# LSDOlab/femo_alpha

Measured on AMD Instinct MI355X. Metric: DOF/s (assembly+solve), forward solve of the RM shell; adjoint-gradient wallclock in adjoint_ms, higher is better.
Workload: dtype f64

## Files before the change

### femo_alpha_amd/backend.py

```python
from __future__ import annotations

import ctypes as C

import numpy as np

from . import _lib
from ._lib import FemoHipError, dptr, iptr
from .mesh import ShellMesh

PENALTY_BETA = 1.0e15


class FemoConvergenceError(FemoHipError):
    """A Krylov solve stopped at maxit short of rtol (status 4; option 'strict')."""


class FemoNotPositiveDefiniteError(FemoHipError):
    """The multifrontal Cholesky met a non-positive pivot (status 5; option 'allow_pivot_repair')."""


class ShellContext:
    VEC_IDS = {"state": 0, "adjoint": 1, "r": 2, "z": 3, "p": 4, "Ap": 5, "b": 6}

    def __init__(self, mesh: ShellMesh, element_wise_material=False, elementwise_pressure=False,
# ... 8 lines not shown
        h = C.c_void_p()
        xyz = np.ascontiguousarray(mesh.nodes, dtype=np.float64)
        cells = np.ascontiguousarray(mesh.cells, dtype=np.int32)
        cp2 = np.ascontiguousarray(mesh.cell_p2, dtype=np.int32)
        if getattr(mesh, "element", "CG2CG1") == "CG2CR1":
            rc = self.lib.femo_create_element(C.byref(h), int(device), mesh.nn, mesh.nel, mesh.nvc, mesh.nP2,
                                              dptr(xyz), iptr(cells), iptr(cp2),
                                              int(self.element_wise_material), int(self.elementwise_pressure), int(nquad),
                                              int(nghost), 1)
        else:
            rc = self.lib.femo_create_ghost(C.byref(h), int(device), mesh.nn, mesh.nel, mesh.nvc, mesh.nP2,
                                            dptr(xyz), iptr(cells), iptr(cp2),
                                            int(self.element_wise_material), int(self.elementwise_pressure), int(nquad),
                                            int(nghost))
        if rc:
            raise FemoHipError(f"femo_create failed ({rc}): {self.lib.femo_last_error(None).decode()}")
        self._h = h
        self.device = int(device)
        self.nghost = int(nghost)
        self.ndof = int(self.lib.femo_ndof(h))
        assert self.ndof == mesh.ndof + self.nghost
        import os
        self.env_options = {}
        for kv in filter(None, (t.strip() for t in os.environ.get("FEMO_OPTIONS", "").split(","))):
            k, sep, v = kv.partition("=")
            try:
                if not sep:
                    raise ValueError
                self.env_options[k.strip()] = float(v)
            except ValueError:
                raise FemoHipError(f"FEMO_OPTIONS: '{kv}' is not of the form option=number (e.g. FEMO_OPTIONS=\"sweep_graph=1,super_tiles=1\")") from None
            self.set_option(k.strip(), self.env_options[k.strip()])
        if self.env_options:
            import sys
            print(f"femo_alpha_amd: FEMO_OPTIONS sets {self.env_options} on this context", file=sys.stderr)

    def _chk(self, rc):
        if rc:
            msg = self.lib.femo_last_error(self._h).decode()
            if rc == 4:
                raise FemoConvergenceError(msg)
            if rc == 5:
                raise FemoNotPositiveDefiniteError(msg)
            raise FemoHipError(msg)

    def set_option(self, key, value):
        self._chk(self.lib.femo_set_option(self._h, key.encode(), float(value)))

    def close(self):
        if getattr(self, "_h", None):
            self.lib.femo_destroy(self._h)
            self._h = None

    def __del__(self):
        try:
            self.close()
        except Exception:
            pass

    @staticmethod
    def _vec(a):
        return np.ascontiguousarray(np.asarray(a, dtype=np.float64).ravel())

    def field_size(self, name):
        n = int(self.lib.femo_field_size(self._h, name.encode()))
        if n < 0:
            raise FemoHipError(f"unknown field '{name}'")
        return n

# ... 156 lines not shown
        wp = None if w is None else dptr(self._vec(w))
        self._chk(self.lib.femo_residual(self._h, wp, dptr(r)))
        return r

    def load_vector(self):
        F = np.empty(self.ndof)
        self._chk(self.lib.femo_load_vector(self._h, dptr(F)))
        return F

    def diagonal(self):
        d = np.empty(self.ndof)
        self._chk(self.lib.femo_diagonal(self._h, dptr(d)))
        return d

    def element_matrices(self, first=0, count=None):
        count = self.mesh.nel - first if count is None else count
        ld = self.mesh.ldof
        Ke = np.empty((count, ld, ld))
        self._chk(self.lib.femo_element_matrices(self._h, first, count, dptr(Ke)))
        return Ke

    def enable_frontal(self, leaf_size=None, plan=None, **options):
        import time
        from .solver.symbolic import build_plan
        leaf_size = self.mesh.recommended_leaf_size() if leaf_size is None else int(leaf_size)
        for k, v in options.items():
            self.set_option(k, v)
        t0 = time.perf_counter()
        plan = self.plan = build_plan(self.mesh, leaf_size) if plan is None else plan
        self.symbolic_s = time.perf_counter() - t0
        i32 = lambda a: np.ascontiguousarray(a, dtype=np.int32)
        i64 = lambda a: np.ascontiguousarray(a, dtype=np.int64)
        level_off = i32(np.concatenate([[0], np.cumsum([len(l) for l in plan.level_nodes])]))
        level_nodes = i32(np.concatenate(plan.level_nodes))
        arrs = dict(nf=i32(plan.nf), npiv=i32(plan.npiv), front_off=i64(plan.front_off), dof_off=i64(plan.dof_off),
                    front_dofs=i32(plan.front_dofs), up_map=i32(plan.up_map), parent=i32(plan.parent), left=i32(plan.left),
                    right=i32(plan.right), level_off=level_off, level_nodes=level_nodes,
                    elem_front=i32(plan.elem_front), elem_map=i32(plan.elem_map))
        p64 = lambda a: a.ctypes.data_as(C.POINTER(C.c_int64))
        self._chk(self.lib.femo_set_frontal_plan(
            self._h, plan.ntree, plan.nlevels, iptr(arrs["nf"]), iptr(arrs["npiv"]), p64(arrs["front_off"]),
            p64(arrs["dof_off"]), iptr(arrs["front_dofs"]), iptr(arrs["up_map"]), iptr(arrs["parent"]), iptr(arrs["left"]),
            iptr(arrs["right"]), iptr(arrs["level_off"]), iptr(arrs["level_nodes"]), iptr(arrs["elem_front"]),
            iptr(arrs["elem_map"])))
        return plan

    def factorize(self):
        self._chk(self.lib.femo_factorize(self._h))
        return self.frontal_info()

    def factorize_profile(self, run=True):
        t = np.zeros(32)
# ... 502 lines not shown
```

### femo_alpha_amd/csrc/symbolic.cpp

```cpp
#include <omp.h>

#include <algorithm>
#include <cmath>
#include <cstdint>
#include <cstdlib>
#include <cstring>
#include <map>
#include <numeric>
#include <string>
#include <vector>

#include "../../include/femo_symbolic.h"

namespace {

struct Plan {
    std::map<std::string, std::vector<int32_t>> i32;
    std::map<std::string, std::vector<int64_t>> i64;
    std::string error;
};

thread_local std::string g_error;

template <class T>
std::vector<T>& put(std::map<std::string, std::vector<T>>& m, const char* name) { return m[name]; }

}

struct femo_plan : Plan {};

extern "C" {

const char* femo_plan_last_error(void) { return g_error.c_str(); }

void femo_plan_free(femo_plan* p) { delete p; }

int femo_plan_build_ex(femo_plan** out, int32_t nel, int32_t nP2, int32_t nV, int32_t npc, int32_t ndpc, const int32_t* cell_p2,
                       const double* cent, const double* cext, const int32_t* cell_dofs, int32_t leaf_size, int32_t min_depth,
                       int32_t axis_rule, double gap_coeff) {
    return femo_plan_build_ex2(out, nel, nP2, nV, npc, ndpc, cell_p2, cent, cext, cell_dofs, leaf_size, min_depth, axis_rule, gap_coeff, 0);
}

int femo_plan_build_ex2(femo_plan** out, int32_t nel, int32_t nP2, int32_t nV, int32_t npc, int32_t ndpc, const int32_t* cell_p2,
                        const double* cent, const double* cext, const int32_t* cell_dofs, int32_t leaf_size, int32_t min_depth,
                        int32_t axis_rule, double gap_coeff, int32_t node_order) {
    if (!out || node_order < 0 || node_order > 1 || nel < 1 || nP2 < 1 || nV < 1 || npc < 1 || ndpc < 1 || !cell_p2 || !cent || !cell_dofs || leaf_size < 1 || min_depth < 0 ||
        axis_rule < 0 || axis_rule > 2 || (axis_rule >= 1 && !cext) || !(gap_coeff >= 0.0)) {
        g_error = "femo_plan_build: bad arguments";
        return 1;
    }
    const int nthreads = std::max(1, std::min(omp_get_max_threads(), 16));
    const int64_t ndof_u = 3 * (int64_t)nP2;
    int32_t fixed_depth = 0;
    while (((int64_t)leaf_size << fixed_depth) < (int64_t)nel) ++fixed_depth;
    fixed_depth = std::max(fixed_depth, min_depth);
    const bool gap_mode = gap_coeff > 0.0;
    constexpr int32_t GAP_NMIN = 128;
    constexpr int32_t AXIS_NMIN = 16;
    std::vector<int32_t> lo{0}, hi{nel}, left{-1}, right{-1}, parent{-1}, depth{0};
    std::vector<int32_t> eorder(nel);
    std::iota(eorder.begin(), eorder.end(), 0);
    struct Scratch { std::vector<int32_t> stamp, first, last, touched; std::vector<long long> diff; };
    std::vector<Scratch> scratch(nthreads);
    {
        std::vector<int32_t> frontier{0};
        while (!frontier.empty()) {
            std::vector<int32_t> split(frontier.size(), -1);
            int bad = 0;
#pragma omp parallel for num_threads(nthreads) schedule(dynamic, 1) reduction(| : bad)
// ... 173 lines not shown
        for (int32_t d = maxdepth; d >= 0; --d) {
            const auto& nodes = by_depth[d];
#pragma omp parallel for num_threads(nthreads) schedule(dynamic, 16)
            for (int64_t k = 0; k < (int64_t)nodes.size(); ++k) {
                const int32_t t = nodes[k];
                std::vector<int32_t> u;
                if (left[t] < 0) {
                    for (int32_t i = lo[t]; i < hi[t]; ++i)
                        for (int a = 0; a < npc; ++a) u.push_back(cell_p2[(int64_t)eorder[i] * npc + a]);
                    std::sort(u.begin(), u.end());
                    u.erase(std::unique(u.begin(), u.end()), u.end());
                } else {
                    const auto &x = bnd[left[t]], &y = bnd[right[t]];
                    u.resize(x.size() + y.size());
                    u.erase(std::set_union(x.begin(), x.end(), y.begin(), y.end(), u.begin()), u.end());
                }
                auto& b = bnd[t];
                b.reserve(u.size());
                for (int32_t n : u)
                    if (owner[n] != t) b.push_back(n);
            }
        }
    }
    if (node_order == 1) {
#pragma omp parallel for num_threads(nthreads) schedule(dynamic, 64)
        for (int32_t t = 0; t < ntree; ++t)
            std::sort(bnd[t].begin(), bnd[t].end(), [&](int32_t x, int32_t y) {
                const int32_t dx = depth[owner[x]], dy = depth[owner[y]];
                return dx != dy ? dx > dy : rank[x] < rank[y];
            });
    }
    std::vector<int64_t> bnd_off(ntree + 1, 0);
    for (int32_t t = 0; t < ntree; ++t) bnd_off[t + 1] = bnd_off[t] + (int64_t)bnd[t].size();
    std::vector<int32_t> bnd_nodes(bnd_off[ntree]);
    for (int32_t t = 0; t < ntree; ++t) std::copy(bnd[t].begin(), bnd[t].end(), bnd_nodes.begin() + bnd_off[t]);
    auto ndofs_of = [&](int32_t n) { return n < nV ? 6 : 3; };
    std::vector<int32_t> npiv(ntree), nf(ntree);
    std::vector<int64_t> dof_off(ntree + 1, 0);
    for (int32_t t = 0; t < ntree; ++t) {
        int64_t a = 0, b = 0;
        for (int64_t i = piv_off[t]; i < piv_off[t + 1]; ++i) a += ndofs_of(piv_nodes[i]);
        for (int32_t n : bnd[t]) b += ndofs_of(n);
        if (a + b > INT32_MAX) { g_error = "front too large"; return 4; }
        npiv[t] = (int32_t)a; nf[t] = (int32_t)(a + b);
        dof_off[t + 1] = dof_off[t] + a + b;
    }
    if (ndof_u + 3 * (int64_t)nV > INT32_MAX) { g_error = "more than 2^31 DOFs"; return 4; }
    std::vector<int32_t> front_dofs(dof_off[ntree]);
#pragma omp parallel for num_threads(nthreads) schedule(dynamic, 64)
    for (int32_t t = 0; t < ntree; ++t) {
        int64_t w = dof_off[t];
        auto emit = [&](int32_t n) {
            for (int c = 0; c < 3; ++c) front_dofs[w++] = 3 * n + c;
            if (n < nV)
                for (int c = 0; c < 3; ++c) front_dofs[w++] = (int32_t)(ndof_u + 3 * (int64_t)n + c);
        };
        for (int64_t i = piv_off[t]; i < piv_off[t + 1]; ++i) emit(piv_nodes[i]);
        for (int32_t n : bnd[t]) emit(n);
    }
// ... 9 lines not shown
#pragma omp parallel for num_threads(nthreads) schedule(dynamic, 16) reduction(| : bad)
    for (int32_t t = 0; t < ntree; ++t) {
        const int32_t n = nf[t];
        const int32_t* fd = front_dofs.data() + dof_off[t];
        std::vector<std::pair<int32_t, int32_t>> srt(n);
        for (int32_t i = 0; i < n; ++i) srt[i] = {fd[i], i};
        std::sort(srt.begin(), srt.end());
        auto find = [&](int32_t dof) {
            auto it = std::lower_bound(srt.begin(), srt.end(), std::make_pair(dof, (int32_t)-1));
            if (it == srt.end() || it->first != dof) { bad |= 1; return -1; }
            return it->second;
        };
        if (left[t] >= 0) {
            for (int32_t ch : {left[t], right[t]})
                for (int64_t i = dof_off[ch] + npiv[ch]; i < dof_off[ch + 1]; ++i) up_map[i] = find(front_dofs[i]);
        } else {
            for (int32_t i = lo[t]; i < hi[t]; ++i) {
                const int32_t e = eorder[i];
                for (int k = 0; k < ndpc; ++k) elem_map[(int64_t)e * ndpc + k] = find(cell_dofs[(int64_t)e * ndpc + k]);
            }
        }
    }
    if (bad) { g_error = "a boundary or element DOF is missing from the front that should hold it"; return 5; }
    int32_t nlevels = 0;
    for (int32_t t = 0; t < ntree; ++t) nlevels = std::max(nlevels, height[t] + 1);
    std::vector<int64_t> level_off(nlevels + 1, 0);
    for (int32_t t = 0; t < ntree; ++t) ++level_off[height[t] + 1];
    for (int32_t h = 0; h < nlevels; ++h) level_off[h + 1] += level_off[h];
    std::vector<int32_t> level_nodes(ntree);
    {
        std::vector<int64_t> fill(level_off.begin(), level_off.end() - 1);
        for (int32_t t = 0; t < ntree; ++t) level_nodes[fill[height[t]]++] = t;
        for (int32_t h = 0; h < nlevels; ++h)
            std::stable_sort(level_nodes.begin() + level_off[h], level_nodes.begin() + level_off[h + 1],
                             [&](int32_t a, int32_t b) { return nf[a] > nf[b]; });
    }
    femo_plan* p = new femo_plan;
    p->i32["lo"] = std::move(lo); p->i32["hi"] = std::move(hi); p->i32["left"] = std::move(left); p->i32["right"] = std::move(right);
    p->i32["parent"] = std::move(parent); p->i32["depth"] = std::move(depth); p->i32["height"] = std::move(height);
    p->i32["eorder"] = std::move(eorder); p->i32["epos"] = std::move(epos); p->i32["owner"] = std::move(owner);
    p->i32["piv_nodes"] = std::move(piv_nodes); p->i64["piv_off"] = std::move(piv_off);
    p->i32["bnd_nodes"] = std::move(bnd_nodes); p->i64["bnd_off"] = std::move(bnd_off);
    p->i32["npiv"] = std::move(npiv); p->i32["nf"] = std::move(nf); p->i64["dof_off"] = std::move(dof_off);
    p->i32["front_dofs"] = std::move(front_dofs); p->i32["up_map"] = std::move(up_map);
    p->i32["elem_front"] = std::move(elem_front); p->i32["elem_map"] = std::move(elem_map);
    p->i32["level_nodes"] = std::move(level_nodes); p->i64["level_off"] = std::move(level_off);
    *out = p;
    return 0;
}

int femo_plan_build(femo_plan** out, int32_t nel, int32_t nP2, int32_t nV, int32_t npc, int32_t ndpc, const int32_t* cell_p2,
                    const double* cent, const int32_t* cell_dofs, int32_t leaf_size, int32_t min_depth) {
    return femo_plan_build_ex(out, nel, nP2, nV, npc, ndpc, cell_p2, cent, nullptr, cell_dofs, leaf_size, min_depth, 0, 0.0);
}

int64_t femo_plan_size(const femo_plan* p, const char* name) {
    if (!p || !name) return -1;
    auto a = p->i32.find(name);
    if (a != p->i32.end()) return (int64_t)a->second.size();
    auto b = p->i64.find(name);
    if (b != p->i64.end()) return (int64_t)b->second.size();
    return -1;
}

int femo_plan_itemsize(const femo_plan* p, const char* name) {
    if (!p || !name) return 0;
    if (p->i32.count(name)) return 4;
    if (p->i64.count(name)) return 8;
    return 0;
// ... 22 lines not shown
```

### femo_alpha_amd/dynamic_rm_shell/plate_sim.py

```python
from __future__ import annotations

import numpy as np

from ..backend import ShellContext


class PlateSim:
    def __init__(self, mesh, E, nu, rho, dt, Nsteps, element_wise_thickness=False, custom_bc_func=None,
                 add_self_weight=False, g_factor=None, quad_deg=3, comm=None, device=0, leaf_size=None, rtol=1e-8):
        import torch
        self.torch = torch
        self.mesh, self.E, self.nu, self.rho, self.dt = mesh, E, nu, rho, dt
        self.Nsteps, self.time_levels = Nsteps, Nsteps + 1
        self.nn, self.nel = mesh.nn, mesh.nel
        self.element_wise_thickness = element_wise_thickness
        self.add_self_weight, self.g_factor, self.quad_deg = add_self_weight, g_factor, quad_deg
        self._sw_weights = mesh.p2_integrals() if (add_self_weight and element_wise_thickness) else None
        ctx = self.ctx = ShellContext(mesh, element_wise_material=element_wise_thickness, device=device)
        ctx.set_field("E", [E]); ctx.set_field("nu", [nu]); ctx.set_field("density", [rho])
        marker = custom_bc_func if custom_bc_func is not None else (lambda x: np.isclose(x[0], 0.0, atol=1e-6))
        self.bc_dofs = mesh.locate_dofs_geometrical(marker)
        ctx.set_strong_dofs(self.bc_dofs)
        npts = (quad_deg + 2) // 2
        if mesh.is_quad and npts < 4:
            ctx.set_strain_quadrature(npts)
        ctx.enable_frontal(leaf_size)
        self.rtol = float(rtol)
        ctx.set_solver(preconditioner=2, rtol=rtol, maxit=50, check_every=1)
        self.a, self.b = 2.0 / dt ** 2, 2.0 / dt
        ctx.set_operator(0.5, self.a)
        self.fe_dofs = ctx.ndof
        self.num_var = ctx.field_size("thickness")
        self.f_history = np.zeros((self.time_levels, 3 * mesh.nn))
        self.t = np.full(self.num_var, 1e-3)
        self.opt_iter = 0
        self.W = None
        self.x_tip, self.cell_tip = None, None
        self._tip = None
        self.tip_disp_history = np.zeros(self.time_levels)
        self.solve_info = []
        self._v = {n: ctx.vec_tensor(n) for n in ("state", "adjoint", "r", "z", "p", "Ap", "b")}

    def update_t(self, t_array):
        self.t = np.asarray(t_array, dtype=np.float64).ravel().copy()
        self.ctx.set_field("thickness", self.t)

    def update_f_history(self, f_history_array):
        self.f_history = np.asarray(f_history_array, dtype=np.float64).reshape(-1, 3 * self.nn)

# ... 225 lines not shown
```

### femo_alpha_amd/parallel.py

```python
from __future__ import annotations

import numpy as np

from .solver.symbolic import analyse, rank_plan

__all__ = ["Comm", "HipEngine", "DistributedShell"]


class Comm:

    def __init__(self, dist=None):
        self.dist = dist if (dist is not None and dist.is_initialized()) else None
        self.rank = self.dist.get_rank() if self.dist else 0
        self.size = self.dist.get_world_size() if self.dist else 1
        self._stage = self.dist is not None and self.dist.get_backend() == "gloo"

    def allreduce_(self, t, op="sum"):
        if self.dist is None:
            return t
        rop = self.dist.ReduceOp.MAX if op == "max" else self.dist.ReduceOp.SUM
        if self._stage and t.is_cuda:
            h = t.cpu()
            self.dist.all_reduce(h, op=rop)
            t.copy_(h)
        else:
            self.dist.all_reduce(t, op=rop)
        return t
# ... 80 lines not shown

    def precond_rest(self):
        self.ctx.dist_precond_rest()

    def direction_apply(self, first):
        self.ctx.dist_direction_apply(first)

    def update(self, x):
        self.ctx.dist_update(x)

    def functionals_partial(self):
        return self.ctx.functionals_partial()

    def dfunctional_vec(self, name, dst):
        self.ctx.dfunctional_vec(name, dst)

    def gradient(self, functional, arg, lam, gglob):
        self.ctx.dist_gradient(functional, arg, lam, gglob)


class DistributedShell:

    def __init__(self, mesh, comm: Comm, bc_marker=None, beta=1.0e15, leaf_size=None, engine_factory=None,
                 element_wise_material=False, device=0, tree=None, nquad=None, strict=True):
        import torch
        self.torch = torch
        self.strict = bool(strict)
        self.mesh, self.comm = mesh, comm
        self.ewm = bool(element_wise_material)
        d = int(np.log2(comm.size))
        leaf_size = mesh.recommended_leaf_size() if leaf_size is None else int(leaf_size)
        self.tree = analyse(mesh, leaf_size, min_depth=d) if tree is None else tree
        self.sub, self.plan, self.info = rank_plan(mesh, self.tree, comm.rank, comm.size)
        self._rule_auto = nquad is None
        self.nquad = mesh.recommended_nquad() if nquad is None else int(nquad)
        factory = engine_factory or (lambda sub, plan, info: HipEngine(sub, plan, info, device=device,
                                                                       element_wise_material=element_wise_material, nquad=self.nquad))
        self.eng = factory(self.sub, self.plan, self.info)
        if bc_marker is not None:
            self.eng.set_penalty_facets(self.sub.penalty_facets(bc_marker), beta)
        self.nl, self.nlev = self.info["n_local_levels"], self.plan.nlevels
        self.ntop = int(self.info["n_top"])
        sel = self.info["cells"] if self.ewm else self.info["vertices"]
        self.eng.dist_setup(self.info["top_local"], comm.size, self.nl, sel)
        self.rtol, self.maxit = 1e-10, 50
        self.factored = False
        self.last = {}
        self._grad_buf = None

    def set_fields(self, thickness=None, E=None, nu=None, density=None, F_solid=None):
        sel = self.info["cells"] if self.ewm else self.info["vertices"]
        for name, v in (("thickness", thickness), ("E", E), ("nu", nu), ("density", density)):
            if v is not None:
                v = np.asarray(v, dtype=np.float64).ravel()
                if name == "nu" and self._rule_auto and not self.mesh.is_quad:
# ... 126 lines not shown
```

### femo_alpha_amd/solver/_native.py

```python
from __future__ import annotations

import ctypes as C

import numpy as np

from .. import _build

_lib = None
_i32p = C.POINTER(C.c_int32)

SIGNATURES = {
    "femo_plan_build": (C.c_int, [C.POINTER(C.c_void_p), C.c_int32, C.c_int32, C.c_int32, C.c_int32, C.c_int32, _i32p,
                                  C.POINTER(C.c_double), _i32p, C.c_int32, C.c_int32]),
    "femo_plan_build_ex": (C.c_int, [C.POINTER(C.c_void_p), C.c_int32, C.c_int32, C.c_int32, C.c_int32, C.c_int32, _i32p,
                                     C.POINTER(C.c_double), C.POINTER(C.c_double), _i32p, C.c_int32, C.c_int32, C.c_int32, C.c_double]),
    "femo_plan_build_ex2": (C.c_int, [C.POINTER(C.c_void_p), C.c_int32, C.c_int32, C.c_int32, C.c_int32, C.c_int32, _i32p,
                                      C.POINTER(C.c_double), C.POINTER(C.c_double), _i32p, C.c_int32, C.c_int32, C.c_int32, C.c_double, C.c_int32]),
    "femo_plan_size": (C.c_int64, [C.c_void_p, C.c_char_p]),
    "femo_plan_itemsize": (C.c_int, [C.c_void_p, C.c_char_p]),
    "femo_plan_get": (C.c_int, [C.c_void_p, C.c_char_p, C.c_void_p, C.c_int64]),
    "femo_plan_free": (None, [C.c_void_p]),
    "femo_plan_last_error": (C.c_char_p, []),
}

ARRAYS = ("lo", "hi", "left", "right", "parent", "depth", "height", "eorder", "epos", "owner", "piv_nodes", "piv_off",
          "bnd_nodes", "bnd_off", "npiv", "nf", "dof_off", "front_dofs", "up_map", "elem_front", "elem_map", "level_nodes",
          "level_off")


def load():
    global _lib
    if _lib is None:
        path = _build.build_symbolic() if _build.symbolic_needs_build() else _build.SYM_LIB
        lib = C.CDLL(path)
        for name, (res, args) in SIGNATURES.items():
            fn = getattr(lib, name)
            fn.restype, fn.argtypes = res, args
        _lib = lib
    return _lib


def plan_arrays(mesh, leaf_size, min_depth=0, axis_rule=0, gap=0.0, node_order=0):
    lib = load()
    cr = getattr(mesh, "element", "") == "CG2CR1"
    nV_lib = mesh.nE if cr else mesh.nV
    cell_p2 = np.ascontiguousarray(mesh.cell_p2, dtype=np.int32)
    cell_dofs = np.ascontiguousarray(mesh.cell_dofs(), dtype=np.int32)
    if cr:
        nV, nE = mesh.nV, mesh.nE
        to_lib = np.concatenate([nE + np.arange(nV), np.arange(nE)]).astype(np.int32)
        from_lib = np.argsort(to_lib).astype(np.int64)
        cell_p2 = np.ascontiguousarray(to_lib[cell_p2])
        cell_dofs = cell_dofs.copy()
        nu = 3 * cell_p2.shape[1]
        cell_dofs[:, :nu] = (3 * np.repeat(cell_p2, 3, axis=1) + np.tile(np.arange(3, dtype=np.int32), cell_p2.shape[1])[None, :])
        cell_dofs = np.ascontiguousarray(cell_dofs, dtype=np.int32)
    xc = mesh.nodes[mesh.cells]
    cent = np.ascontiguousarray(xc.mean(axis=1), dtype=np.float64)
    cext = np.ascontiguousarray(xc.max(axis=1) - xc.min(axis=1), dtype=np.float64)
    h = C.c_void_p()
    dp = C.POINTER(C.c_double)
    rc = lib.femo_plan_build_ex2(C.byref(h), mesh.nel, mesh.nP2, nV_lib, cell_p2.shape[1], cell_dofs.shape[1],
                                 cell_p2.ctypes.data_as(_i32p), cent.ctypes.data_as(dp), cext.ctypes.data_as(dp),
                                 cell_dofs.ctypes.data_as(_i32p), int(leaf_size), int(min_depth), int(axis_rule), float(gap), int(node_order))
    if rc:
        msg = lib.femo_plan_last_error().decode()
        raise ValueError(msg) if rc == 2 else RuntimeError(msg)
    try:
        out = {}
        for name in ARRAYS:
            n, isz = lib.femo_plan_size(h, name.encode()), lib.femo_plan_itemsize(h, name.encode())
            a = np.empty(n, dtype=np.int32 if isz == 4 else np.int64)
            if lib.femo_plan_get(h, name.encode(), a.ctypes.data_as(C.c_void_p), a.nbytes):
                raise RuntimeError(lib.femo_plan_last_error().decode())
            out[name] = a
    finally:
        lib.femo_plan_free(h)
    out["elem_map"] = out["elem_map"].reshape(mesh.nel, -1)
    if cr:
        fd = out["front_dofs"].astype(np.int64)
        isu = fd < mesh.ndof_u
        fd[isu] = 3 * from_lib[fd[isu] // 3] + fd[isu] % 3
        out["front_dofs"] = fd.astype(out["front_dofs"].dtype)
        for k in ("piv_nodes", "bnd_nodes"):
            out[k] = from_lib[out[k]].astype(out[k].dtype)
        out["owner"] = out["owner"][to_lib]
    return out
# ... 1 lines not shown
```

### femo_alpha_amd/solver/symbolic.py

```python
from __future__ import annotations

import numpy as np

from ..mesh import ShellMesh

__all__ = ["FrontalPlan", "Tree", "analyse", "build_plan", "rank_plan"]


class FrontalPlan:

    def summary(self):
        nf, npv = self.nf, self.npiv
        flops = float(np.sum(npv.astype(np.float64) * nf.astype(np.float64) ** 2
                             - npv.astype(np.float64) ** 2 * nf + npv.astype(np.float64) ** 3 / 3.0))
        return dict(fronts=int(self.ntree), levels=int(self.nlevels), leaves=int(self.nleaves),
                    max_front=int(nf.max()), max_pivots=int(npv.max()),
                    front_doubles=int(self.front_off[-1]), front_GB=float(self.front_off[-1] * 8 / 1e9),
                    factor_doubles=int(np.sum(nf.astype(np.int64) * npv)), factor_gflop=flops / 1e9)


class Tree:
    """Nested-dissection tree over the elements with, per tree node, the P2 nodes it eliminates
    (``piv_nodes``) and the ancestor-owned P2 nodes its subtree touches (``bnd_nodes``)."""


def _node_dofs(nodes, nV, ndof_u, rot=None):
    nodes = np.asarray(nodes, dtype=np.int64)
    if rot is not None:
        r0, nr = rot
        is_r = (nodes >= r0) & (nodes < r0 + nr)
        cnt = np.where(is_r, 6, 3)
        off = np.concatenate([[0], np.cumsum(cnt)])
        out = np.empty(off[-1], dtype=np.int64)
        base = off[:-1]
        for c in range(3):
            out[base + c] = 3 * nodes + c
        rb, rn = base[is_r], nodes[is_r] - r0
        for c in range(3):
            out[rb + 3 + c] = ndof_u + 3 * rn + c
        return out
    is_v = nodes < nV
    cnt = np.where(is_v, 6, 3)
    off = np.concatenate([[0], np.cumsum(cnt)])
    out = np.empty(off[-1], dtype=np.int64)
    base = off[:-1]
    for c in range(3):
        out[base + c] = 3 * nodes + c
    vb = base[is_v]
    vn = nodes[is_v]
    for c in range(3):
        out[vb + 3 + c] = ndof_u + 3 * vn + c
    return out


def _tree_from_native(A) -> Tree:
    T = Tree()
    for k in ("lo", "hi", "left", "right", "parent", "depth", "height", "eorder", "epos", "owner"):
        setattr(T, k, A[k].astype(np.int64))
    T.ntree = T.lo.size
    po, bo = A["piv_off"], A["bnd_off"]
    pn, bn = A["piv_nodes"].astype(np.int64), A["bnd_nodes"].astype(np.int64)
    T.piv_nodes = [pn[po[t]:po[t + 1]] for t in range(T.ntree)]
    T.bnd_nodes = [bn[bo[t]:bo[t + 1]] for t in range(T.ntree)]
    return T


AXIS_RULE = 2
GAP = 0.75
NODE_ORDER = 1
GAP_NMIN = 128
AXIS_NMIN = 16


def analyse(mesh, leaf_size=12, min_depth=0, impl="native", axis_rule=None, gap=None, node_order=None) -> Tree:
    axis_rule = AXIS_RULE if axis_rule is None else int(axis_rule)
    gap = GAP if gap is None else float(gap)
    node_order = NODE_ORDER if node_order is None else int(node_order)
    if impl == "native":
        from . import _native
        return _tree_from_native(_native.plan_arrays(mesh, leaf_size, min_depth, axis_rule, gap, node_order))
    if getattr(mesh, "element", "") == "CG2CR1":
        raise NotImplementedError("the numpy twin of the analysis knows the vertex-rotation layouts only; CG2CR1 goes through the native library")
    nel, nP2 = mesh.nel, mesh.nP2
    xc = mesh.nodes[mesh.cells]
    cent = xc.mean(axis=1)
    cext = xc.max(axis=1) - xc.min(axis=1)
    eorder = np.arange(nel)
    lo_l, hi_l, left_l, right_l, parent_l, depth_l = [0], [nel], [-1], [-1], [-1], [0]
    fixed_depth = 0
    while (leaf_size << fixed_depth) < nel:
        fixed_depth += 1
    fixed_depth = max(fixed_depth, min_depth)
    frontier = [0]
    while frontier:
        nxt = []
        for t in frontier:
            lo, hi = lo_l[t], hi_l[t]
            n = hi - lo
            want = depth_l[t] < fixed_depth if gap > 0 else (n > leaf_size or depth_l[t] < min_depth)
            if not want:
                continue
            if n < 2:
                if depth_l[t] < min_depth:
# ... 87 lines not shown
    T.owner = owner
    height = np.zeros(T.ntree, dtype=np.int64)
    order_bu = np.argsort(-T.depth, kind="stable")
    for t in order_bu:
        if not is_leaf[t]:
            height[t] = 1 + max(height[T.left[t]], height[T.right[t]])
    T.height = height
    ord_owner = np.argsort(owner, kind="stable")
    cnt = np.bincount(owner, minlength=T.ntree)
    st = np.concatenate([[0], np.cumsum(cnt)])
    T.piv_nodes = [ord_owner[st[t]:st[t + 1]] for t in range(T.ntree)]
    bnd = [None] * T.ntree
    for t in order_bu:
        if is_leaf[t]:
            touched = np.unique(mesh.cell_p2[eorder[T.lo[t]:T.hi[t]]])
            bnd[t] = touched[owner[touched] != t]
        else:
            u = np.union1d(bnd[T.left[t]], bnd[T.right[t]])
            bnd[t] = u[owner[u] != t]
    if node_order == 1:
        nc = np.zeros((nP2, 3))
        np.add.at(nc, mesh.cell_p2.ravel(), np.repeat(cent, mesh.cell_p2.shape[1], axis=0))
        nc /= np.maximum(np.bincount(mesh.cell_p2.ravel(), minlength=nP2), 1)[:, None]
        rank = np.zeros(nP2, dtype=np.int64)
        for t in range(T.ntree):
            p = T.piv_nodes[t]
            if p.size > 1:
                ax = int(np.argmax(nc[p].max(axis=0) - nc[p].min(axis=0)))
                p = p[np.argsort(nc[p, ax], kind="stable")]
                T.piv_nodes[t] = p
            rank[p] = np.arange(p.size)
        for t in range(T.ntree):
            b = bnd[t]
            bnd[t] = b[np.lexsort((rank[b], -T.depth[owner[b]]))]
    T.bnd_nodes = bnd
    return T


def _assemble_plan(dof_lists, npiv, parent, left, right, level_of, elem_front, elem_dofs):
    ntree = len(dof_lists)
    plan = FrontalPlan()
    plan.ntree = ntree
    plan.npiv = np.asarray(npiv, dtype=np.int32)
    plan.nf = np.array([len(d) for d in dof_lists], dtype=np.int32)
    plan.parent = np.asarray(parent, dtype=np.int32)
    plan.left, plan.right = np.asarray(left, dtype=np.int32), np.asarray(right, dtype=np.int32)
    plan.nleaves = int(np.sum(plan.left < 0))
    plan.dof_off = np.concatenate([[0], np.cumsum(plan.nf.astype(np.int64))])
    plan.front_dofs = (np.concatenate(dof_lists) if ntree else np.zeros(0)).astype(np.int32)
    plan.front_off = np.concatenate([[0], np.cumsum(plan.nf.astype(np.int64) ** 2)])
    sorters = {}

    def positions(t, dofs):
        if t not in sorters:
            fd = np.asarray(dof_lists[t])
            o = np.argsort(fd, kind="stable")
            sorters[t] = (fd[o], o)
        fs, o = sorters[t]
        k = np.searchsorted(fs, dofs)
# ... 15 lines not shown
        es = order[bounds[t]:bounds[t + 1]]
        if es.size:
            elem_map[es] = positions(t, elem_dofs[es].ravel()).reshape(es.size, -1)
    plan.elem_map = elem_map
    level_of = np.asarray(level_of)
    plan.nlevels = int(level_of.max()) + 1
    plan.height = level_of.astype(np.int32)
    lev_nodes = [np.nonzero(level_of == h)[0] for h in range(plan.nlevels)]
    plan.level_nodes = [ln[np.argsort(-plan.nf[ln], kind="stable")].astype(np.int32) for ln in lev_nodes]
    return plan


def _plan_from_native(A) -> FrontalPlan:
    plan = FrontalPlan()
    plan.ntree = int(A["nf"].size)
    for k in ("npiv", "nf", "parent", "left", "right", "front_dofs", "up_map", "elem_front", "elem_map", "height", "eorder"):
        setattr(plan, k, A[k])
    plan.nleaves = int(np.sum(plan.left < 0))
    plan.dof_off = A["dof_off"]
    plan.front_off = np.concatenate([[0], np.cumsum(plan.nf.astype(np.int64) ** 2)])
    lo = A["level_off"]
    plan.nlevels = int(lo.size - 1)
    plan.level_nodes = [A["level_nodes"][lo[h]:lo[h + 1]] for h in range(plan.nlevels)]
    return plan


def build_plan(mesh, leaf_size=12, impl="native", axis_rule=None, gap=None, node_order=None) -> FrontalPlan:
    axis_rule = AXIS_RULE if axis_rule is None else int(axis_rule)
    gap = GAP if gap is None else float(gap)
    node_order = NODE_ORDER if node_order is None else int(node_order)
    if impl == "native":
        from . import _native
        return _plan_from_native(_native.plan_arrays(mesh, leaf_size, 0, axis_rule, gap, node_order))
    T = analyse(mesh, leaf_size, impl="python", axis_rule=axis_rule, gap=gap, node_order=node_order)
    nV, ndof_u = mesh.nV, mesh.ndof_u
    seq = [a for t in range(T.ntree) for a in (T.piv_nodes[t], T.bnd_nodes[t])]
    lens = np.array([len(a) for a in seq], dtype=np.int64)
    nodes_all = np.concatenate(seq).astype(np.int64) if seq else np.zeros(0, np.int64)
    csum = np.concatenate([[0], np.cumsum(np.where(nodes_all < nV, 6, 3))])
    ends = np.cumsum(lens)
    ndofs_seg = csum[ends] - csum[ends - lens]
    dofs_all = _node_dofs(nodes_all, nV, ndof_u)
    seg_off = np.concatenate([[0], np.cumsum(ndofs_seg)])
    dof_lists = [dofs_all[seg_off[2 * t]:seg_off[2 * t + 2]] for t in range(T.ntree)]
    npiv = ndofs_seg[0::2]
    leaf_of_pos = np.zeros(mesh.nel, dtype=np.int64)
    for t in np.nonzero(T.left < 0)[0]:
        leaf_of_pos[T.lo[t]:T.hi[t]] = t
    plan = _assemble_plan(dof_lists, npiv, T.parent, T.left, T.right, T.height, leaf_of_pos[T.epos], mesh.cell_dofs())
    plan.eorder = T.eorder.astype(np.int32)
    return plan


def rank_plan(mesh, T: Tree, rank, nranks):
    return _rank_plan(mesh, T, rank, nranks)


def _rank_plan(mesh, T: Tree, rank, nranks):
    d = int(np.log2(nranks))
    if 2 ** d != nranks:
        raise ValueError("number of ranks must be a power of two")
    roots = np.nonzero(T.depth == d)[0]
    roots = roots[np.argsort(T.lo[roots], kind="stable")]
    if roots.size != nranks or np.any(T.depth[T.left < 0] < d):
        raise ValueError("tree is not deep enough for this many ranks")
    root = int(roots[rank])
    nVg, ndof_ug = mesh.nV, mesh.ndof_u
    cr = getattr(mesh, "element", "") == "CG2CR1"
    rot_g = (mesh.nV, mesh.nE) if cr else None
    cells_g = np.sort(T.eorder[T.lo[root]:T.hi[root]])
    verts_g = np.unique(mesh.cells[cells_g])
    g2l_v = -np.ones(mesh.nn, dtype=np.int64)
    g2l_v[verts_g] = np.arange(verts_g.size)
# ... 71 lines not shown
```

### include/femo_symbolic.h

```cpp
#ifndef FEMO_SYMBOLIC_H
#define FEMO_SYMBOLIC_H
#include <stdint.h>
#ifdef __cplusplus
extern "C" {
#endif

typedef struct femo_plan femo_plan;

int femo_plan_build(femo_plan** out, int32_t nel, int32_t nP2, int32_t nV, int32_t npc, int32_t ndpc, const int32_t* cell_p2,
                    const double* cent, const int32_t* cell_dofs, int32_t leaf_size, int32_t min_depth);
int femo_plan_build_ex(femo_plan** out, int32_t nel, int32_t nP2, int32_t nV, int32_t npc, int32_t ndpc, const int32_t* cell_p2,
                       const double* cent, const double* cext, const int32_t* cell_dofs, int32_t leaf_size, int32_t min_depth,
                       int32_t axis_rule, double gap_coeff);
int femo_plan_build_ex2(femo_plan** out, int32_t nel, int32_t nP2, int32_t nV, int32_t npc, int32_t ndpc, const int32_t* cell_p2,
                        const double* cent, const double* cext, const int32_t* cell_dofs, int32_t leaf_size, int32_t min_depth,
                        int32_t axis_rule, double gap_coeff, int32_t node_order);
int64_t femo_plan_size(const femo_plan* p, const char* name);
int femo_plan_itemsize(const femo_plan* p, const char* name);
int femo_plan_get(const femo_plan* p, const char* name, void* dst, int64_t nbytes);
void femo_plan_free(femo_plan* p);
const char* femo_plan_last_error(void);

#ifdef __cplusplus
}
#endif
#endif
```

Measured before the change: 61.85 million.

## Delay small pivot tails to parent fronts to cut factorization panel count

Adds a symbolic-analysis pass that moves the last few pivot nodes of each front to its parent whenever a level's largest pivot block just spills into an extra 128-wide panel. The aim is to remove one panel step from every front at that level in the batched multifrontal Cholesky, provided parent panel counts do not grow and total flops rise by no more than 1%. It is enabled by default with TAIL_MAX=32 through enable_frontal, and it makes the affected fronts larger and changes the elimination order.

After: 62.99 million (median of 6 runs). +1.8%, better.

```diff
diff --git a/femo_alpha_amd/backend.py b/femo_alpha_amd/backend.py
--- a/femo_alpha_amd/backend.py
+++ b/femo_alpha_amd/backend.py
@@ -54,6 +54,7 @@
         assert self.ndof == mesh.ndof + self.nghost
         import os
         self.env_options = {}
+        self.tail_max = None
         for kv in filter(None, (t.strip() for t in os.environ.get("FEMO_OPTIONS", "").split(","))):
             k, sep, v = kv.partition("=")
             try:
@@ -77,6 +78,11 @@
             raise FemoHipError(msg)
 
     def set_option(self, key, value):
+        if key == "tail_max":
+            if float(value) < 0 or float(value) != int(value):
+                raise FemoHipError("option 'tail_max' takes a non-negative whole number of DOFs (0 = off)")
+            self.tail_max = int(value)
+            return
         self._chk(self.lib.femo_set_option(self._h, key.encode(), float(value)))
 
     def close(self):
@@ -279,12 +285,13 @@
 
     def enable_frontal(self, leaf_size=None, plan=None, **options):
         import time
-        from .solver.symbolic import build_plan
+        from .solver.symbolic import TAIL_MAX, build_plan
         leaf_size = self.mesh.recommended_leaf_size() if leaf_size is None else int(leaf_size)
         for k, v in options.items():
             self.set_option(k, v)
         t0 = time.perf_counter()
-        plan = self.plan = build_plan(self.mesh, leaf_size) if plan is None else plan
+        tail_max = TAIL_MAX if self.tail_max is None else self.tail_max
+        plan = self.plan = build_plan(self.mesh, leaf_size, tail_max=tail_max) if plan is None else plan
         self.symbolic_s = time.perf_counter() - t0
         i32 = lambda a: np.ascontiguousarray(a, dtype=np.int32)
         i64 = lambda a: np.ascontiguousarray(a, dtype=np.int64)
diff --git a/femo_alpha_amd/csrc/symbolic.cpp b/femo_alpha_amd/csrc/symbolic.cpp
--- a/femo_alpha_amd/csrc/symbolic.cpp
+++ b/femo_alpha_amd/csrc/symbolic.cpp
@@ -44,7 +44,13 @@
 int femo_plan_build_ex2(femo_plan** out, int32_t nel, int32_t nP2, int32_t nV, int32_t npc, int32_t ndpc, const int32_t* cell_p2,
                         const double* cent, const double* cext, const int32_t* cell_dofs, int32_t leaf_size, int32_t min_depth,
                         int32_t axis_rule, double gap_coeff, int32_t node_order) {
-    if (!out || node_order < 0 || node_order > 1 || nel < 1 || nP2 < 1 || nV < 1 || npc < 1 || ndpc < 1 || !cell_p2 || !cent || !cell_dofs || leaf_size < 1 || min_depth < 0 ||
+    return femo_tail_delay_plan_build(out, nel, nP2, nV, npc, ndpc, cell_p2, cent, cext, cell_dofs, leaf_size, min_depth, axis_rule, gap_coeff, node_order, 0);
+}
+
+int femo_tail_delay_plan_build(femo_plan** out, int32_t nel, int32_t nP2, int32_t nV, int32_t npc, int32_t ndpc, const int32_t* cell_p2,
+                               const double* cent, const double* cext, const int32_t* cell_dofs, int32_t leaf_size, int32_t min_depth,
+                               int32_t axis_rule, double gap_coeff, int32_t node_order, int32_t tail_max) {
+    if (!out || tail_max < 0 || node_order < 0 || node_order > 1 || nel < 1 || nP2 < 1 || nV < 1 || npc < 1 || ndpc < 1 || !cell_p2 || !cent || !cell_dofs || leaf_size < 1 || min_depth < 0 ||
         axis_rule < 0 || axis_rule > 2 || (axis_rule >= 1 && !cext) || !(gap_coeff >= 0.0)) {
         g_error = "femo_plan_build: bad arguments";
         return 1;
@@ -264,6 +270,94 @@
             }
         }
     }
+    auto ndofs_of = [&](int32_t n) { return n < nV ? 6 : 3; };
+    int32_t nlevels = 0;
+    for (int32_t t = 0; t < ntree; ++t) nlevels = std::max(nlevels, height[t] + 1);
+    std::vector<int64_t> td_dofs(nlevels, 0), td_flops3(2, 0);
+    std::vector<int32_t> td_saved(nlevels, 0);
+    if (tail_max > 0) {
+        constexpr int64_t NBO = 128;
+        std::vector<int64_t> np(ntree, 0), nfv(ntree, 0);
+        std::vector<std::vector<int32_t>> piv(ntree), by_height(nlevels);
+        auto flops3 = [](int64_t a, int64_t f) { return 3 * a * f * f - 3 * a * a * f + a * a * a; };
+        int64_t F0 = 0;
+        std::vector<int64_t> lev_max(nlevels, 0);
+        for (int32_t t = 0; t < ntree; ++t) {
+            piv[t].assign(piv_nodes.begin() + piv_off[t], piv_nodes.begin() + piv_off[t + 1]);
+            for (int32_t n : piv[t]) np[t] += ndofs_of(n);
+            nfv[t] = np[t];
+            for (int32_t n : bnd[t]) nfv[t] += ndofs_of(n);
+            F0 += flops3(np[t], nfv[t]);
+            by_height[height[t]].push_back(t);
+            lev_max[height[t]] = std::max(lev_max[height[t]], np[t]);
+        }
+        int64_t F = F0;
+        auto panels = [&](int64_t m) { return (m + NBO - 1) / NBO; };
+        struct Move { int32_t t; int32_t nnodes; int64_t dofs; };
+        std::vector<int64_t> add(ntree, 0);
+        std::vector<std::vector<int32_t>> recv(ntree);
+        for (int32_t h = 0; h + 1 < nlevels; ++h) {
+            const int64_t P = panels(lev_max[h]);
+            if (P < 2) continue;
+            const int64_t keep = NBO * (P - 1);
+            std::vector<Move> mv;
+            std::vector<int32_t> par;
+            bool ok = true;
+            for (int32_t t : by_height[h]) {
+                const int64_t tail = np[t] - keep;
+                if (tail <= 0) continue;
+                if (tail > tail_max || parent[t] < 0 || depth[t] <= min_depth) { ok = false; break; }
+                int64_t got = 0;
+                int32_t cnt = 0;
+                for (int64_t i = (int64_t)piv[t].size() - 1; got < tail; --i) { got += ndofs_of(piv[t][i]); ++cnt; }
+                mv.push_back({t, cnt, got});
+                if (add[parent[t]] == 0) par.push_back(parent[t]);
+                add[parent[t]] += got;
+            }
+            int64_t Fn = F;
+            if (ok) {
+                std::vector<int64_t> grown(lev_max);
+                for (int32_t p : par) grown[height[p]] = std::max(grown[height[p]], np[p] + add[p]);
+                for (int32_t p : par)
+                    if (panels(grown[height[p]]) > panels(lev_max[height[p]])) ok = false;
+                for (const Move& m : mv) Fn += flops3(np[m.t] - m.dofs, nfv[m.t]) - flops3(np[m.t], nfv[m.t]);
+                for (int32_t p : par) Fn += flops3(np[p] + add[p], nfv[p] + add[p]) - flops3(np[p], nfv[p]);
+                if (100 * Fn > 101 * F0) ok = false;
+            }
+            if (ok) {
+                for (const Move& m : mv) {
+                    const int32_t t = m.t, p = parent[t];
+                    for (size_t i = piv[t].size() - m.nnodes; i < piv[t].size(); ++i) {
+                        const int32_t n = piv[t][i];
+                        owner[n] = p; recv[p].push_back(n); bnd[t].push_back(n);
+                    }
+                    piv[t].resize(piv[t].size() - m.nnodes);
+                    std::sort(bnd[t].begin(), bnd[t].end());
+                    np[t] -= m.dofs;
+                    td_dofs[h] += m.dofs;
+                }
+                for (int32_t p : par) {
+                    recv[p].insert(recv[p].end(), piv[p].begin(), piv[p].end());
+                    piv[p].swap(recv[p]);
+                    recv[p].clear();
+                    np[p] += add[p]; nfv[p] += add[p];
+                    lev_max[height[p]] = std::max(lev_max[height[p]], np[p]);
+                }
+                lev_max[h] = 0;
+                for (int32_t t : by_height[h]) lev_max[h] = std::max(lev_max[h], np[t]);
+                td_saved[h] = (int32_t)(P - panels(lev_max[h]));
+                F = Fn;
+            }
+            for (int32_t p : par) add[p] = 0;
+        }
+        td_flops3[0] = F0; td_flops3[1] = F;
+        for (int32_t t = 0; t < ntree; ++t) {
+            piv_off[t + 1] = piv_off[t] + (int64_t)piv[t].size();
+            std::copy(piv[t].begin(), piv[t].end(), piv_nodes.begin() + piv_off[t]);
+            if (node_order == 1)
+                for (size_t i = 0; i < piv[t].size(); ++i) rank[piv[t][i]] = (int32_t)i;
+        }
+    }
     if (node_order == 1) {
 #pragma omp parallel for num_threads(nthreads) schedule(dynamic, 64)
         for (int32_t t = 0; t < ntree; ++t)
@@ -276,7 +370,6 @@
     for (int32_t t = 0; t < ntree; ++t) bnd_off[t + 1] = bnd_off[t] + (int64_t)bnd[t].size();
     std::vector<int32_t> bnd_nodes(bnd_off[ntree]);
     for (int32_t t = 0; t < ntree; ++t) std::copy(bnd[t].begin(), bnd[t].end(), bnd_nodes.begin() + bnd_off[t]);
-    auto ndofs_of = [&](int32_t n) { return n < nV ? 6 : 3; };
     std::vector<int32_t> npiv(ntree), nf(ntree);
     std::vector<int64_t> dof_off(ntree + 1, 0);
     for (int32_t t = 0; t < ntree; ++t) {
@@ -332,8 +425,6 @@
         }
     }
     if (bad) { g_error = "a boundary or element DOF is missing from the front that should hold it"; return 5; }
-    int32_t nlevels = 0;
-    for (int32_t t = 0; t < ntree; ++t) nlevels = std::max(nlevels, height[t] + 1);
     std::vector<int64_t> level_off(nlevels + 1, 0);
     for (int32_t t = 0; t < ntree; ++t) ++level_off[height[t] + 1];
     for (int32_t h = 0; h < nlevels; ++h) level_off[h + 1] += level_off[h];
@@ -355,6 +446,8 @@
     p->i32["front_dofs"] = std::move(front_dofs); p->i32["up_map"] = std::move(up_map);
     p->i32["elem_front"] = std::move(elem_front); p->i32["elem_map"] = std::move(elem_map);
     p->i32["level_nodes"] = std::move(level_nodes); p->i64["level_off"] = std::move(level_off);
+    p->i64["tail_delay_dofs"] = std::move(td_dofs); p->i32["tail_delay_saved"] = std::move(td_saved);
+    p->i64["tail_delay_flops3"] = std::move(td_flops3);
     *out = p;
     return 0;
 }
diff --git a/femo_alpha_amd/dynamic_rm_shell/plate_sim.py b/femo_alpha_amd/dynamic_rm_shell/plate_sim.py
--- a/femo_alpha_amd/dynamic_rm_shell/plate_sim.py
+++ b/femo_alpha_amd/dynamic_rm_shell/plate_sim.py
@@ -7,7 +7,7 @@
 
 class PlateSim:
     def __init__(self, mesh, E, nu, rho, dt, Nsteps, element_wise_thickness=False, custom_bc_func=None,
-                 add_self_weight=False, g_factor=None, quad_deg=3, comm=None, device=0, leaf_size=None, rtol=1e-8):
+                 add_self_weight=False, g_factor=None, quad_deg=3, comm=None, device=0, leaf_size=None, rtol=1e-8, tail_max=None):
         import torch
         self.torch = torch
         self.mesh, self.E, self.nu, self.rho, self.dt = mesh, E, nu, rho, dt
@@ -24,7 +24,7 @@
         npts = (quad_deg + 2) // 2
         if mesh.is_quad and npts < 4:
             ctx.set_strain_quadrature(npts)
-        ctx.enable_frontal(leaf_size)
+        ctx.enable_frontal(leaf_size, **({} if tail_max is None else dict(tail_max=tail_max)))
         self.rtol = float(rtol)
         ctx.set_solver(preconditioner=2, rtol=rtol, maxit=50, check_every=1)
         self.a, self.b = 2.0 / dt ** 2, 2.0 / dt
diff --git a/femo_alpha_amd/parallel.py b/femo_alpha_amd/parallel.py
--- a/femo_alpha_amd/parallel.py
+++ b/femo_alpha_amd/parallel.py
@@ -2,7 +2,7 @@
 
 import numpy as np
 
-from .solver.symbolic import analyse, rank_plan
+from .solver.symbolic import TAIL_MAX, analyse, rank_plan
 
 __all__ = ["Comm", "HipEngine", "DistributedShell"]
 
@@ -129,7 +129,7 @@
 class DistributedShell:
 
     def __init__(self, mesh, comm: Comm, bc_marker=None, beta=1.0e15, leaf_size=None, engine_factory=None,
-                 element_wise_material=False, device=0, tree=None, nquad=None, strict=True):
+                 element_wise_material=False, device=0, tree=None, nquad=None, strict=True, tail_max=None):
         import torch
         self.torch = torch
         self.strict = bool(strict)
@@ -137,7 +137,11 @@
         self.ewm = bool(element_wise_material)
         d = int(np.log2(comm.size))
         leaf_size = mesh.recommended_leaf_size() if leaf_size is None else int(leaf_size)
-        self.tree = analyse(mesh, leaf_size, min_depth=d) if tree is None else tree
+        if tail_max is None:
+            import os
+            env = dict(kv.split("=", 1) for kv in os.environ.get("FEMO_OPTIONS", "").replace(" ", "").split(",") if "=" in kv)
+            tail_max = int(float(env["tail_max"])) if "tail_max" in env else TAIL_MAX
+        self.tree = analyse(mesh, leaf_size, min_depth=d, tail_max=tail_max) if tree is None else tree
         self.sub, self.plan, self.info = rank_plan(mesh, self.tree, comm.rank, comm.size)
         self._rule_auto = nquad is None
         self.nquad = mesh.recommended_nquad() if nquad is None else int(nquad)
diff --git a/femo_alpha_amd/solver/_native.py b/femo_alpha_amd/solver/_native.py
--- a/femo_alpha_amd/solver/_native.py
+++ b/femo_alpha_amd/solver/_native.py
@@ -23,9 +23,13 @@
     "femo_plan_last_error": (C.c_char_p, []),
 }
 
+TAIL_DELAY_SIGNATURES = {
+    "femo_tail_delay_plan_build": (C.c_int, SIGNATURES["femo_plan_build_ex2"][1] + [C.c_int32]),
+}
+
 ARRAYS = ("lo", "hi", "left", "right", "parent", "depth", "height", "eorder", "epos", "owner", "piv_nodes", "piv_off",
           "bnd_nodes", "bnd_off", "npiv", "nf", "dof_off", "front_dofs", "up_map", "elem_front", "elem_map", "level_nodes",
-          "level_off")
+          "level_off", "tail_delay_dofs", "tail_delay_saved", "tail_delay_flops3")
 
 
 def load():
@@ -33,14 +37,14 @@
     if _lib is None:
         path = _build.build_symbolic() if _build.symbolic_needs_build() else _build.SYM_LIB
         lib = C.CDLL(path)
-        for name, (res, args) in SIGNATURES.items():
+        for name, (res, args) in {**SIGNATURES, **TAIL_DELAY_SIGNATURES}.items():
             fn = getattr(lib, name)
             fn.restype, fn.argtypes = res, args
         _lib = lib
     return _lib
 
 
-def plan_arrays(mesh, leaf_size, min_depth=0, axis_rule=0, gap=0.0, node_order=0):
+def plan_arrays(mesh, leaf_size, min_depth=0, axis_rule=0, gap=0.0, node_order=0, tail_max=0):
     lib = load()
     cr = getattr(mesh, "element", "") == "CG2CR1"
     nV_lib = mesh.nE if cr else mesh.nV
@@ -60,9 +64,10 @@
     cext = np.ascontiguousarray(xc.max(axis=1) - xc.min(axis=1), dtype=np.float64)
     h = C.c_void_p()
     dp = C.POINTER(C.c_double)
-    rc = lib.femo_plan_build_ex2(C.byref(h), mesh.nel, mesh.nP2, nV_lib, cell_p2.shape[1], cell_dofs.shape[1],
-                                 cell_p2.ctypes.data_as(_i32p), cent.ctypes.data_as(dp), cext.ctypes.data_as(dp),
-                                 cell_dofs.ctypes.data_as(_i32p), int(leaf_size), int(min_depth), int(axis_rule), float(gap), int(node_order))
+    args = (C.byref(h), mesh.nel, mesh.nP2, nV_lib, cell_p2.shape[1], cell_dofs.shape[1],
+            cell_p2.ctypes.data_as(_i32p), cent.ctypes.data_as(dp), cext.ctypes.data_as(dp),
+            cell_dofs.ctypes.data_as(_i32p), int(leaf_size), int(min_depth), int(axis_rule), float(gap), int(node_order))
+    rc = lib.femo_plan_build_ex2(*args) if tail_max is None else lib.femo_tail_delay_plan_build(*args, int(tail_max))
     if rc:
         msg = lib.femo_plan_last_error().decode()
         raise ValueError(msg) if rc == 2 else RuntimeError(msg)
diff --git a/femo_alpha_amd/solver/symbolic.py b/femo_alpha_amd/solver/symbolic.py
--- a/femo_alpha_amd/solver/symbolic.py
+++ b/femo_alpha_amd/solver/symbolic.py
@@ -13,10 +13,16 @@
         nf, npv = self.nf, self.npiv
         flops = float(np.sum(npv.astype(np.float64) * nf.astype(np.float64) ** 2
                              - npv.astype(np.float64) ** 2 * nf + npv.astype(np.float64) ** 3 / 3.0))
-        return dict(fronts=int(self.ntree), levels=int(self.nlevels), leaves=int(self.nleaves),
-                    max_front=int(nf.max()), max_pivots=int(npv.max()),
-                    front_doubles=int(self.front_off[-1]), front_GB=float(self.front_off[-1] * 8 / 1e9),
-                    factor_doubles=int(np.sum(nf.astype(np.int64) * npv)), factor_gflop=flops / 1e9)
+        out = dict(fronts=int(self.ntree), levels=int(self.nlevels), leaves=int(self.nleaves),
+                   max_front=int(nf.max()), max_pivots=int(npv.max()),
+                   front_doubles=int(self.front_off[-1]), front_GB=float(self.front_off[-1] * 8 / 1e9),
+                   factor_doubles=int(np.sum(nf.astype(np.int64) * npv)), factor_gflop=flops / 1e9)
+        td = getattr(self, "tail_delay", None)
+        if td is not None and int(np.sum(td["saved"])):
+            f0, f1 = td["flops3"]
+            out.update(delayed_dofs=int(np.sum(td["dofs"])), panels_saved={int(h): int(s) for h, s in enumerate(td["saved"]) if s},
+                       delay_flop_change=float(f1 - f0) / float(f0))
+        return out
 
 
 class Tree:
@@ -62,7 +68,12 @@
     pn, bn = A["piv_nodes"].astype(np.int64), A["bnd_nodes"].astype(np.int64)
     T.piv_nodes = [pn[po[t]:po[t + 1]] for t in range(T.ntree)]
     T.bnd_nodes = [bn[bo[t]:bo[t + 1]] for t in range(T.ntree)]
+    T.tail_delay = _tail_delay_native(A)
     return T
+
+
+def _tail_delay_native(A):
+    return dict(dofs=A["tail_delay_dofs"], saved=A["tail_delay_saved"], flops3=tuple(int(v) for v in A["tail_delay_flops3"]))
 
 
 AXIS_RULE = 2
@@ -72,13 +83,13 @@
 AXIS_NMIN = 16
 
 
-def analyse(mesh, leaf_size=12, min_depth=0, impl="native", axis_rule=None, gap=None, node_order=None) -> Tree:
+def analyse(mesh, leaf_size=12, min_depth=0, impl="native", axis_rule=None, gap=None, node_order=None, tail_max=0) -> Tree:
     axis_rule = AXIS_RULE if axis_rule is None else int(axis_rule)
     gap = GAP if gap is None else float(gap)
     node_order = NODE_ORDER if node_order is None else int(node_order)
     if impl == "native":
         from . import _native
-        return _tree_from_native(_native.plan_arrays(mesh, leaf_size, min_depth, axis_rule, gap, node_order))
+        return _tree_from_native(_native.plan_arrays(mesh, leaf_size, min_depth, axis_rule, gap, node_order, tail_max))
     if getattr(mesh, "element", "") == "CG2CR1":
         raise NotImplementedError("the numpy twin of the analysis knows the vertex-rotation layouts only; CG2CR1 goes through the native library")
     nel, nP2 = mesh.nel, mesh.nP2
@@ -212,19 +223,86 @@
         nc = np.zeros((nP2, 3))
         np.add.at(nc, mesh.cell_p2.ravel(), np.repeat(cent, mesh.cell_p2.shape[1], axis=0))
         nc /= np.maximum(np.bincount(mesh.cell_p2.ravel(), minlength=nP2), 1)[:, None]
-        rank = np.zeros(nP2, dtype=np.int64)
         for t in range(T.ntree):
             p = T.piv_nodes[t]
             if p.size > 1:
                 ax = int(np.argmax(nc[p].max(axis=0) - nc[p].min(axis=0)))
-                p = p[np.argsort(nc[p, ax], kind="stable")]
-                T.piv_nodes[t] = p
-            rank[p] = np.arange(p.size)
+                T.piv_nodes[t] = p[np.argsort(nc[p, ax], kind="stable")]
+    T.tail_delay = _tail_delay(T, bnd, mesh.nV, int(min_depth), int(tail_max))
+    if node_order == 1:
+        rank = np.zeros(nP2, dtype=np.int64)
+        for t in range(T.ntree):
+            rank[T.piv_nodes[t]] = np.arange(T.piv_nodes[t].size)
         for t in range(T.ntree):
             b = bnd[t]
             bnd[t] = b[np.lexsort((rank[b], -T.depth[owner[b]]))]
     T.bnd_nodes = bnd
     return T
+
+
+NBO = 128
+TAIL_MAX = 32
+
+
+def _tail_delay(T, bnd, nV, min_depth, tail_max):
+    nlev = int(T.height.max()) + 1
+    dofs, saved = np.zeros(nlev, dtype=np.int64), np.zeros(nlev, dtype=np.int32)
+    if tail_max <= 0:
+        return dict(dofs=dofs, saved=saved, flops3=(0, 0))
+    nd = lambda a: int(np.where(np.asarray(a) < nV, 6, 3).sum())
+    flops3 = lambda a, f: 3 * a * f * f - 3 * a * a * f + a * a * a
+    panels = lambda m: (m + NBO - 1) // NBO
+    npv = [nd(T.piv_nodes[t]) for t in range(T.ntree)]
+    nfv = [npv[t] + nd(bnd[t]) for t in range(T.ntree)]
+    F0 = F = sum(flops3(a, f) for a, f in zip(npv, nfv))
+    by_height = [np.nonzero(T.height == h)[0] for h in range(nlev)]
+    lev_max = [max(npv[t] for t in by_height[h]) for h in range(nlev)]
+    for h in range(nlev - 1):
+        P = panels(lev_max[h])
+        if P < 2:
+            continue
+        keep = NBO * (P - 1)
+        mv, add, ok = [], {}, True
+        for t in by_height[h]:
+            tail = npv[t] - keep
+            if tail <= 0:
+                continue
+            if tail > tail_max or T.parent[t] < 0 or T.depth[t] <= min_depth:
+                ok = False
+                break
+            w = np.where(T.piv_nodes[t] < nV, 6, 3)[::-1].cumsum()
+            cnt = int(np.searchsorted(w, tail)) + 1
+            mv.append((int(t), cnt, int(w[cnt - 1])))
+            add[int(T.parent[t])] = add.get(int(T.parent[t]), 0) + int(w[cnt - 1])
+        if not ok:
+            continue
+        grown = list(lev_max)
+        for p, a in add.items():
+            grown[T.height[p]] = max(grown[T.height[p]], npv[p] + a)
+        if any(panels(grown[T.height[p]]) > panels(lev_max[T.height[p]]) for p in add):
+            continue
+        Fn = F + sum(flops3(npv[t] - d, nfv[t]) - flops3(npv[t], nfv[t]) for t, _, d in mv) \
+               + sum(flops3(npv[p] + a, nfv[p] + a) - flops3(npv[p], nfv[p]) for p, a in add.items())
+        if 100 * Fn > 101 * F0:
+            continue
+        recv = {p: [] for p in add}
+        for t, cnt, d in mv:
+            p = int(T.parent[t])
+            D = T.piv_nodes[t][-cnt:]
+            T.owner[D] = p
+            recv[p].append(D)
+            bnd[t] = np.sort(np.concatenate([bnd[t], D]))
+            T.piv_nodes[t] = T.piv_nodes[t][:-cnt]
+            npv[t] -= d
+            dofs[h] += d
+        for p, a in add.items():
+            T.piv_nodes[p] = np.concatenate(recv[p] + [T.piv_nodes[p]])
+            npv[p] += a; nfv[p] += a
+            lev_max[T.height[p]] = max(lev_max[T.height[p]], npv[p])
+        lev_max[h] = max(npv[t] for t in by_height[h])
+        saved[h] = P - panels(lev_max[h])
+        F = Fn
+    return dict(dofs=dofs, saved=saved, flops3=(int(F0), int(F)))
 
 
 def _assemble_plan(dof_lists, npiv, parent, left, right, level_of, elem_front, elem_dofs):
@@ -286,17 +364,18 @@
     lo = A["level_off"]
     plan.nlevels = int(lo.size - 1)
     plan.level_nodes = [A["level_nodes"][lo[h]:lo[h + 1]] for h in range(plan.nlevels)]
+    plan.tail_delay = _tail_delay_native(A)
     return plan
 
 
-def build_plan(mesh, leaf_size=12, impl="native", axis_rule=None, gap=None, node_order=None) -> FrontalPlan:
+def build_plan(mesh, leaf_size=12, impl="native", axis_rule=None, gap=None, node_order=None, tail_max=0) -> FrontalPlan:
     axis_rule = AXIS_RULE if axis_rule is None else int(axis_rule)
     gap = GAP if gap is None else float(gap)
     node_order = NODE_ORDER if node_order is None else int(node_order)
     if impl == "native":
         from . import _native
-        return _plan_from_native(_native.plan_arrays(mesh, leaf_size, 0, axis_rule, gap, node_order))
-    T = analyse(mesh, leaf_size, impl="python", axis_rule=axis_rule, gap=gap, node_order=node_order)
+        return _plan_from_native(_native.plan_arrays(mesh, leaf_size, 0, axis_rule, gap, node_order, tail_max))
+    T = analyse(mesh, leaf_size, impl="python", axis_rule=axis_rule, gap=gap, node_order=node_order, tail_max=tail_max)
     nV, ndof_u = mesh.nV, mesh.ndof_u
     seq = [a for t in range(T.ntree) for a in (T.piv_nodes[t], T.bnd_nodes[t])]
     lens = np.array([len(a) for a in seq], dtype=np.int64)
@@ -313,6 +392,7 @@
         leaf_of_pos[T.lo[t]:T.hi[t]] = t
     plan = _assemble_plan(dof_lists, npiv, T.parent, T.left, T.right, T.height, leaf_of_pos[T.epos], mesh.cell_dofs())
     plan.eorder = T.eorder.astype(np.int32)
+    plan.tail_delay = T.tail_delay
     return plan
 
 
diff --git a/include/femo_symbolic.h b/include/femo_symbolic.h
--- a/include/femo_symbolic.h
+++ b/include/femo_symbolic.h
@@ -15,6 +15,9 @@
 int femo_plan_build_ex2(femo_plan** out, int32_t nel, int32_t nP2, int32_t nV, int32_t npc, int32_t ndpc, const int32_t* cell_p2,
                         const double* cent, const double* cext, const int32_t* cell_dofs, int32_t leaf_size, int32_t min_depth,
                         int32_t axis_rule, double gap_coeff, int32_t node_order);
+int femo_tail_delay_plan_build(femo_plan** out, int32_t nel, int32_t nP2, int32_t nV, int32_t npc, int32_t ndpc, const int32_t* cell_p2,
+                               const double* cent, const double* cext, const int32_t* cell_dofs, int32_t leaf_size, int32_t min_depth,
+                               int32_t axis_rule, double gap_coeff, int32_t node_order, int32_t tail_max);
 int64_t femo_plan_size(const femo_plan* p, const char* name);
 int femo_plan_itemsize(const femo_plan* p, const char* name);
 int femo_plan_get(const femo_plan* p, const char* name, void* dst, int64_t nbytes);
```
